# zellerlab/GECCO

Hardware: AMD Instinct MI355X
Metric: genes/sec CRF decode (windowed fwd-bwd marginals + Viterbi) (higher is better)
Workload: dtype f64

## Files before the change

gecco_amd/csrc/crf_kernels.hip:

```cpp
#include "crf_device.hpp"
#include "crf_vd_short.hpp"

namespace gecco {
namespace {

typedef double f64x2 __attribute__((ext_vector_type(2)));

__device__ __forceinline__ double wave_shr1_zero(double v) {
    int lo = __double2loint(v), hi = __double2hiint(v);
    lo = __builtin_amdgcn_update_dpp(0, lo, 0x138, 0xF, 0xF, true);
    hi = __builtin_amdgcn_update_dpp(0, hi, 0x138, 0xF, 0xF, true);
    return __hiloint2double(hi, lo);
}

__device__ __forceinline__ double max_nocanon(double a, double b) {
    double r;
    asm("v_max_f64 %0, %1, %2" : "=v"(r) : "v"(a), "v"(b));
    return r;
}

__device__ __forceinline__ int xcd_remap(int orig, int nwg) {
    const int xcd = orig & 7, q = nwg >> 3, r = nwg & 7;
    const int base = xcd < r ? xcd * (q + 1) : r * (q + 1) + (xcd - r) * q;
    return base + (orig >> 3);
}

__device__ __forceinline__ void store_wt(double *p, double v) {
    __hip_atomic_store(reinterpret_cast<unsigned long long *>(p), static_cast<unsigned long long>(__double_as_longlong(v)),
                       __ATOMIC_RELAXED, __HIP_MEMORY_SCOPE_AGENT);
}

__device__ __forceinline__ double lds_read1(const double *p) {
    return __longlong_as_double(static_cast<long long>(
        __hip_atomic_load(reinterpret_cast<const unsigned long long *>(p), __ATOMIC_RELAXED, __HIP_MEMORY_SCOPE_WORKGROUP)));
}

__device__ __forceinline__ void rescale_pair(double &u, double &v) {
    int ex;
    (void)frexp(fmax(u, v), &ex);
    u = ldexp(u, -ex);
    v = ldexp(v, -ex);
}


constexpr int kGatherUnroll = 8;

template <int WMAX, int NT, int TT, bool EXACT>
struct WinSmem {
    static constexpr int JMAX = TT == 1 ? 2 : TT;
    static constexpr int CAP = TT == 1 ? NT + WMAX - 1 : TT * NT;
    static constexpr int CMAX = EXACT ? CAP / WMAX + 3 : CAP + 2;
    f64x2 ef[2 * CAP];
    uint32_t ginfo[CAP];
    f64x2 carry[NT / 64][WMAX];
    int32_t cslot[CMAX];
    int32_t cgene[CMAX];
    int32_t cn[CMAX];
};

struct SlotInfo {
    int gene;
    bool start_ok;
};

template <class Smem>
__device__ __forceinline__ SlotInfo slot_lookup(const Smem &sm, int cnt, int q, int S, int W, int step) {
    SlotInfo r{-1, false};
    if (q < 0 || q >= S) return r;
    int lo = 0, hi = cnt - 1;
    while (lo < hi) {
        const int mid = (lo + hi + 1) >> 1;
        if (sm.cslot[mid] <= q) lo = mid; else hi = mid - 1;
    }
    const int pos = q - sm.cslot[lo];
    const int np = sm.cslot[lo + 1] - sm.cslot[lo];
    const int n = sm.cn[lo];
    const int gl = pos - ((np - n) >> 1);
    if (gl >= 0 && gl < n) r.gene = sm.cgene[lo] + gl;
    r.start_ok = (pos + W <= np) && (step == 1 || pos % step == 0);
    return r;
}

__device__ __forceinline__ void state_scores_l2(const int32_t *__restrict__ attr_id,
                                                const double2 *__restrict__ wtab2, int n_attrs, int lo, int hi,
                                                double &s0, double &s1) {
    for (int base = lo; base < hi; base += kGatherUnroll) {
        int a[kGatherUnroll];
#pragma unroll
        for (int u = 0; u < kGatherUnroll; ++u) a[u] = base + u < hi ? attr_id[base + u] : -1;
        double2 w[kGatherUnroll];
#pragma unroll
        for (int u = 0; u < kGatherUnroll; ++u) w[u] = unsigned(a[u]) < unsigned(n_attrs) ? wtab2[a[u]] : make_double2(0.0, 0.0);
#pragma unroll
        for (int u = 0; u < kGatherUnroll; ++u) {
            s0 += w[u].x;
            s1 += w[u].y;
        }
    }
}

typedef int i32x4 __attribute__((ext_vector_type(4)));

__device__ __forceinline__ void state_scores_buf(__amdgpu_buffer_rsrc_t ra, __amdgpu_buffer_rsrc_t rw, uint32_t off,
                                                 uint32_t cnt, double &s0, double &s1) {
    for (uint32_t base = 0; base < cnt; base += kGatherUnroll) {
        int a[kGatherUnroll];
#pragma unroll
        for (int u = 0; u < kGatherUnroll; ++u)
            a[u] = __builtin_amdgcn_raw_buffer_load_b32(ra, int((off + base + u) << 2), 0, 0);
        i32x4 w[kGatherUnroll];
#pragma unroll
        for (int u = 0; u < kGatherUnroll; ++u) {
            const uint32_t wo = base + u < cnt ? min(uint32_t(a[u]), 0x0FFFFFFFu) << 4 : 0xFFFFFFF0u;
            w[u] = __builtin_amdgcn_raw_buffer_load_b128(rw, int(wo), 0, 0);
        }
#pragma unroll
        for (int u = 0; u < kGatherUnroll; ++u) {
            s0 += __hiloint2double(w[u].y, w[u].x);
            s1 += __hiloint2double(w[u].w, w[u].z);
        }
    }
}

template <int WMAX, bool EXACT, bool RESCALE, int NT, int TT, bool LEAN = false, bool SMALL = false>
__device__ __forceinline__ void windowed_tile(const WinArgs &P, WinSmem<WMAX, NT, TT, EXACT> &sm, const int tile) {
    using Smem = WinSmem<WMAX, NT, TT, EXACT>;
    constexpr int JMAX = Smem::JMAX;
    constexpr bool RATIO = !RESCALE && EXACT;
    const int W = EXACT ? WMAX : P.W;
    const int tid = threadIdx.x, lane = tid & 63, wave = tid >> 6;
    const int OUT = NT - (W - 1);
    const int ns = TT * OUT + 2 * (W - 1);
    const int q0 = tile * (TT * OUT) - (W - 1);

    const int4 td = P.all_regular ? make_int4(0, 0, 0, 1) : P.tile_desc[tile];
    int gene[JMAX];
    bool start[JMAX];
#pragma unroll
    for (int j = 0; j < JMAX; ++j) {
        gene[j] = -1;
        start[j] = false;
    }
    if (td.w & 1) {
#pragma unroll
        for (int j = 0; j < JMAX; ++j) {
            const int sl = tid + j * NT, q = q0 + sl;
            if (sl < ns && q >= 0 && q < P.S) {
                gene[j] = q + td.x;
                start[j] = (reinterpret_cast<const uint32_t *>(P.start_bits)[q >> 5] >> (q & 31)) & 1u;
            }
        }
    } else {
        const int cnt = td.z - td.y + 1;
        for (int j = tid; j <= cnt; j += NT) {
            sm.cslot[j] = P.c_slot[td.y + j];
            if (j < cnt) {
                sm.cgene[j] = P.c_gene[td.y + j];
                sm.cn[j] = P.c_n[td.y + j];
            }
        }
        __syncthreads();
#pragma unroll
        for (int j = 0; j < JMAX; ++j) {
            const int sl = tid + j * NT;
            if (sl < ns) {
                const SlotInfo si = slot_lookup(sm, cnt, q0 + sl, P.S, W, P.step);
                gene[j] = si.gene;
                start[j] = si.start_ok;
            }
        }
    }

    const uint32_t nnz = SMALL ? uint32_t(P.csr_end) : uint32_t(P.gene_ptr[P.n_genes]);
    const int g_first = (td.w & 1) ? (q0 > 0 ? q0 : 0) + td.x : P.c_gene[td.y];
    const uint32_t lo_tile = SMALL ? uint32_t(P.csr_begin) : uint32_t(P.gene_ptr[g_first]);
    const uint64_t abytes = uint64_t(nnz - lo_tile) << 2;
    const __amdgpu_buffer_rsrc_t ra = __builtin_amdgcn_make_buffer_rsrc(
        const_cast<int32_t *>(P.attr_id + lo_tile), 0, abytes > 0xFFFFFFFFull ? 0xFFFFFFFFu : uint32_t(abytes), 0x00020000);
    const __amdgpu_buffer_rsrc_t rw =
        __builtin_amdgcn_make_buffer_rsrc(const_cast<double2 *>(P.wtab2), 0, uint32_t(P.A) << 4, 0x00020000);

    double sc0[JMAX], sc1[JMAX];
#pragma unroll
    for (int j = 0; j < JMAX; ++j) sc0[j] = sc1[j] = 0.0;
    if (td.w & 1) {
        uint32_t lo[JMAX], hi[JMAX];
#pragma unroll
        for (int j = 0; j < JMAX; ++j) {
            lo[j] = hi[j] = 0;
            if (gene[j] >= 0) {
                lo[j] = uint32_t(P.gene_ptr[gene[j]]);
                hi[j] = uint32_t(P.gene_ptr[gene[j] + 1]);
            }
        }
        const int q_end = min(q0 + ns, P.S);
        const uint32_t hi_tile = SMALL ? uint32_t(P.csr_end) : uint32_t(P.gene_ptr[q_end + td.x]);
        const uint32_t n_attr = hi_tile - lo_tile;
        constexpr int SBASE = (Smem::CAP + 1) / 2;
        constexpr int APL = (2 * Smem::CAP - SBASE) / NT;
        constexpr int SCAP = APL * NT;
        static_assert(APL >= 1, "parking area smaller than one round of the workgroup");
        f64x2 *park = sm.ef + SBASE;
#pragma unroll 1
        for (uint32_t base = 0; base < n_attr; base += SCAP) {
            int id[APL];
#pragma unroll
            for (int a = 0; a < APL; ++a) id[a] = __builtin_amdgcn_raw_buffer_load_b32(ra, int((base + a * NT + tid) << 2), 0, 0);
            i32x4 w[APL];
#pragma unroll
            for (int a = 0; a < APL; ++a) {
                const uint32_t wo = min(uint32_t(id[a]), 0x0FFFFFFFu) << 4;
                w[a] = __builtin_amdgcn_raw_buffer_load_b128(rw, int(wo), 0, 0);
            }
#pragma unroll
            for (int a = 0; a < APL; ++a)
                park[a * NT + tid] = f64x2{__hiloint2double(w[a].y, w[a].x), __hiloint2double(w[a].w, w[a].z)};
            __syncthreads();
            const uint32_t c0 = lo_tile + base, c1 = c0 + SCAP;
#pragma unroll
            for (int j = 0; j < JMAX; ++j) {
                const f64x2 *k = park + (max(lo[j], c0) - c0);
                const f64x2 *const e = park + (min(hi[j], c1) - c0);
                for (; k < e && hi[j] > c0; ++k) {
                    const f64x2 v = *k;
                    sc0[j] += v.x;
                    sc1[j] += v.y;
                }
            }
            if (base + SCAP < n_attr) __syncthreads();
        }
        if (!RATIO && n_attr > 0) __syncthreads();
    } else {
        uint32_t off[JMAX], cnt[JMAX];
#pragma unroll
        for (int j = 0; j < JMAX; ++j) {
            int lo = 0, hi = 0;
            if (gene[j] >= 0) {
                lo = P.gene_ptr[gene[j]];
                hi = P.gene_ptr[gene[j] + 1];
            }
            off[j] = uint32_t(lo) - lo_tile;
            cnt[j] = uint32_t(hi - lo);
        }
        int ids[JMAX][kGatherUnroll];
#pragma unroll
        for (int j = 0; j < JMAX; ++j)
            if (TT > 1 || j == 0 || wave == 0) {
#pragma unroll
                for (int u = 0; u < kGatherUnroll; ++u)
                    ids[j][u] = __builtin_amdgcn_raw_buffer_load_b32(ra, int((off[j] + u) << 2), 0, 0);
            }
#pragma unroll
        for (int j = 0; j < JMAX; ++j) {
            if (TT > 1 || j == 0 || wave == 0) {
                double s0 = 0.0, s1 = 0.0;
                i32x4 w[kGatherUnroll];
#pragma unroll
                for (int u = 0; u < kGatherUnroll; ++u) {
                    const uint32_t wo = uint32_t(u) < cnt[j] ? min(uint32_t(ids[j][u]), 0x0FFFFFFFu) << 4 : 0xFFFFFFF0u;
                    w[u] = __builtin_amdgcn_raw_buffer_load_b128(rw, int(wo), 0, 0);
                }
#pragma unroll
                for (int u = 0; u < kGatherUnroll; ++u) {
                    s0 += __hiloint2double(w[u].y, w[u].x);
                    s1 += __hiloint2double(w[u].w, w[u].z);
                }
                if (cnt[j] > uint32_t(kGatherUnroll))
                    state_scores_buf(ra, rw, off[j] + kGatherUnroll, cnt[j] - kGatherUnroll, s0, s1);
                sc0[j] = s0;
                sc1[j] = s1;
            }
        }
    }
    double *rr = reinterpret_cast<double *>(sm.ef);
#pragma unroll
    for (int j = 0; j < JMAX; ++j) {
        if (TT > 1 || j == 0 || wave == 0) {
            const int sl = tid + j * NT;
            const double s0 = sc0[j], s1 = sc1[j];
            if (sl >= W - 1 && sl < TT * OUT + (W - 1) && gene[j] >= 0) {
                if (P.state_out) reinterpret_cast<f64x2 *>(P.state_out)[gene[j]] = P.label ? f64x2{s0, s1} : f64x2{s1, s0};
            }
            const double d = s1 - s0;
            if (sl < ns) {
                if (RATIO) {
                    const double r = mu_exp_tab(d, P.rtab, P.expc);
                    rr[sl] = __hiloint2double(__double2hiint(r) | (start[j] ? int(0x80000000u) : 0), __double2loint(r));
                    if (!(td.w & 1)) sm.ginfo[sl] = uint32_t(gene[j] + 1);
                } else {
                    const double e = exp_neg(fabs(d), P.expc);
                    const double e1 = d > 0.0 ? 1.0 : e;
                    sm.ef[sl] = f64x2{d > 0.0 ? e : 1.0, P.mu01 * e1};
                    sm.ginfo[sl] = (start[j] ? 0x80000000u : 0u) | uint32_t(gene[j] + 1);
                }
            }
        }
    }
    if (P.dstate_out) {
#pragma unroll
        for (int j = 0; j < JMAX; ++j) {
            if (TT > 1 || j == 0 || wave == 0) {
                const int sl = tid + j * NT;
                if (sl >= W - 1 && sl < TT * OUT + (W - 1) && gene[j] >= 0) {
                    const double d = sc1[j] - sc0[j];
                    const double dd = __hiloint2double(__double2hiint(d) ^ (P.label ? 0 : int(0x80000000u)), __double2loint(d));
                    store_wt(P.dstate_out + gene[j], dd);
                }
            }
        }
    }
    __syncthreads();

    const uint32_t rmask = P.rescale_mask;
    const double rho = P.rho;
#pragma unroll 1
    for (int ph = 0; ph < TT; ++ph) {
        if (SMALL && ph > 0 && q0 + (W - 1) + ph * OUT >= P.S) break;
        const int sbase = ph * OUT + tid;
        bool my_start = false;
        int my_gene;
        if (RATIO) {
            const int q = q0 + sbase;
            my_gene = (td.w & 1) ? ((q >= 0 && q < P.S) ? q + td.x : -1) : int(sm.ginfo[sbase]) - 1;
        } else {
            const uint32_t gi = sm.ginfo[sbase];
            my_start = gi >> 31;
            my_gene = int(gi & 0x7fffffffu) - 1;
        }
        const f64x2 *ef = sm.ef + sbase;
        if constexpr (RATIO) {
            const double *rrs = rr + sbase;
            double A1[WMAX];
            const double r0 = lds_read1(rrs);
            double a0 = 1.0, a1 = fabs(r0) * P.kappa_over_mu01;
            A1[0] = a1;
#pragma unroll
            for (int k = 1; k < WMAX; ++k) {
                if (EXACT || k < W) {
                    const double r = fabs(lds_read1(rrs + k));
                    const double t = a0 + a1;
                    a1 = fma(a1, rho, a0) * r;
                    a0 = t;
                    A1[k] = a1;
                }
            }
            asm volatile("" ::: "memory");
            double z = fma(a1, P.inv_kappa, a0);
            const bool renorm = __builtin_amdgcn_ballot_w64(!(z < P.ratio_zmax)) != 0;
            auto pair_of = [&](double r, double &e0, double &f) {
                const bool pos = r > P.mu01;
                const double rc = fmin(r, 1.0e300);
                double q = __builtin_amdgcn_rcp(rc);
                q = fma(fma(-rc, q, 1.0), q, q);
                e0 = pos ? P.mu01 * q : 1.0;
                f = pos ? P.mu01 : r;
            };
            if (renorm) {
                double e0, f;
                pair_of(fabs(r0), e0, f);
                a0 = e0;
                a1 = f * P.kappa_over_mu01;
                A1[0] = a1;
#pragma unroll
                for (int k = 1; k < WMAX; ++k) {
                    if (EXACT || k < W) {
                        pair_of(fabs(rrs[k]), e0, f);
                        const double t = a0 + a1;
                        a1 = fma(a1, rho, a0) * f;
                        a0 = t * e0;
                        A1[k] = a1;
                    }
                }
                z = fma(a1, P.inv_kappa, a0);
            }
            double b0, b1;
            {
                double r = __builtin_amdgcn_rcp(z);
                r = fma(fma(-z, r, 1.0), r, r);
                b0 = __double2hiint(r0) < 0 ? r : 0.0;
                b1 = b0 * P.inv_kappa;
            }
            double R = 0.0;
            double *carry = reinterpret_cast<double *>(&sm.carry[0][0]);
            if (!renorm) {
                double rcur = W > 1 ? lds_read1(rrs + (W - 1)) : 0.0;
#pragma unroll
                for (int k = WMAX - 1; k >= 0; --k) {
                    if (EXACT || k < W) {
                        double rnext = 0.0;
                        if (k > 1) rnext = lds_read1(rrs + (k - 1));
                        const double cand = A1[k] * b1;
                        if (k < W - 1) {
                            if (lane == 63 && wave < NT / 64 - 1) carry[wave * WMAX + k] = R;
                            R = wave_shr1_zero(R);
                        }
                        R = max_nocanon(R, cand);
                        if (k > 0) {
                            const double u = fabs(rcur) * b1;
                            b1 = fma(u, rho, b0);
                            b0 = b0 + u;
                        }
                        rcur = rnext;
                    }
                }
            } else {
#pragma unroll
                for (int k = WMAX - 1; k >= 0; --k) {
                    if (EXACT || k < W) {
                        const double cand = A1[k] * b1;
                        if (k < W - 1) {
                            if (lane == 63 && wave < NT / 64 - 1) carry[wave * WMAX + k] = R;
                            R = wave_shr1_zero(R);
                        }
                        R = max_nocanon(R, cand);
                        if (k > 0) {
                            double e0, f;
                            pair_of(fabs(rrs[k]), e0, f);
                            const double cc = e0 * b0, u = f * b1;
                            b0 = cc + u;
                            b1 = fma(u, rho, cc);
                        }
                    }
                }
            }
            __syncthreads();
            if (wave > 0 && lane < W - 1) {
                int t2 = tid;
                if (LEAN) asm volatile("" : "+v"(t2));
                R = fmax(R, carry[((t2 >> 6) - 1) * WMAX + (t2 & 63)]);
            }
            R = fmin(R, 1.0);
            if (tid >= W - 1 && my_gene >= 0) store_wt(P.p_out + my_gene, R);
        } else if constexpr (!RESCALE) {
            double A1[WMAX];
            double a0, a1;
            {
                const f64x2 c = ef[0];
                a0 = c.x;
                a1 = fabs(c.y) * P.kappa_over_mu01;
            }
            A1[0] = a1;
#pragma unroll
            for (int k = 1; k < WMAX; ++k) {
                if (EXACT || k < W) {
                    const f64x2 c = ef[k];
                    const double t = a0 + a1;
                    a1 = fma(a1, rho, a0) * fabs(c.y);
                    a0 = t * c.x;
                    A1[k] = a1;
                }
            }
            asm volatile("" ::: "memory");

            double b0, b1;
            {
                const double z = fma(a1, P.inv_kappa, a0);
                double r = __builtin_amdgcn_rcp(z);
                r = fma(fma(-z, r, 1.0), r, r);
                b0 = my_start ? r : 0.0;
                b1 = b0 * P.inv_kappa;
            }
            double R = 0.0;
            double *carry = reinterpret_cast<double *>(&sm.carry[0][0]);
#pragma unroll
            for (int k = WMAX - 1; k >= 0; --k) {
                if (EXACT || k < W) {
                    const double cand = A1[k] * b1;
                    if (k < W - 1) {
                        if (lane == 63 && wave < NT / 64 - 1) carry[wave * WMAX + k] = R;
                        R = wave_shr1_zero(R);
                    }
                    R = max_nocanon(R, cand);
                    if (k > 0) {
                        const f64x2 c = ef[k];
                        const double cc = c.x * b0, u = fabs(c.y) * b1;
                        b0 = cc + u;
                        b1 = fma(u, rho, cc);
                    }
                }
            }
            __syncthreads();
            if (wave > 0 && lane < W - 1) R = fmax(R, carry[(wave - 1) * WMAX + lane]);
            R = fmin(R, 1.0);
            if (tid >= W - 1 && my_gene >= 0) P.p_out[my_gene] = R;
        } else {
            double A0[WMAX], A1[WMAX];
            double a0, a1;
            {
                const f64x2 c = ef[0];
                a0 = c.x;
                a1 = c.y * P.kappa_over_mu01;
            }
            A0[0] = a0;
            A1[0] = a1;
#pragma unroll
            for (int k = 1; k < WMAX; ++k) {
                if (EXACT || k < W) {
                    const f64x2 c = ef[k];
                    const double t = a0 + a1;
                    const double n1 = fma(a1, rho, a0) * c.y;
                    a0 = t * c.x;
                    a1 = n1;
                    if ((rmask >> k) & 1u) rescale_pair(a0, a1);
                    A0[k] = a0;
                    A1[k] = a1;
                }
            }
            asm volatile("" ::: "memory");
            double b0 = 1.0, b1 = P.inv_kappa;
            double Rx = 0.0, Ry = 0.0;
#pragma unroll
            for (int k = WMAX - 1; k >= 0; --k) {
                if (EXACT || k < W) {
                    const double x = A1[k] * b1;
                    const double y = A0[k] * b0;
                    if (k < W - 1) {
                        if (lane == 63 && wave < NT / 64 - 1) sm.carry[wave][k] = f64x2{Rx, Ry};
                        Rx = wave_shr1_zero(Rx);
                        Ry = wave_shr1_zero(Ry);
                    }
                    const bool take = my_start && (x * Ry >= Rx * y);
                    Rx = take ? x : Rx;
                    Ry = take ? y : Ry;
                    if (k > 0) {
                        const f64x2 c = ef[k];
                        const double cc = c.x * b0, u = c.y * b1;
                        b0 = cc + u;
                        b1 = fma(u, rho, cc);
                        if ((rmask >> k) & 1u) rescale_pair(b0, b1);
                    }
                }
            }
            __syncthreads();
            if (wave > 0 && lane < W - 1) {
                const f64x2 c = sm.carry[wave - 1][lane];
                if (c.x * Ry > Rx * c.y || (Rx == 0.0 && Ry == 0.0)) {
                    Rx = c.x;
                    Ry = c.y;
                }
            }
            if (tid >= W - 1 && my_gene >= 0) P.p_out[my_gene] = (Rx + Ry > 0.0) ? Rx / (Rx + Ry) : 0.0;
        }
        if (TT > 1) __syncthreads();
    }
}

template <int WMAX, bool EXACT, bool RESCALE, int NT, int TT>
__global__ void __launch_bounds__(NT, (RESCALE ? (WMAX <= 20 ? 5 : 3) : (WMAX <= 20 ? (TT <= 2 ? 8 : 5) : 3))) crf_windowed_l2(const WinArgs P) {
    __shared__ WinSmem<WMAX, NT, TT, EXACT> sm;
    windowed_tile<WMAX, EXACT, RESCALE, NT, TT>(P, sm, xcd_remap(blockIdx.x, P.ntiles));
}

__global__ void __launch_bounds__(kWinThreads, 4) crf_windowed_small_l2(const WinArgs P) {
    __shared__ WinSmem<20, kWinThreads, 2, true> sm;
    windowed_tile<20, true, false, kWinThreads, 2, false, true>(P, sm, 0);
}

struct PipeArgs {
    const int32_t *gene_ptr, *attr_id;
    const double2 *wtab2;
    const int32_t *c_slot, *c_gene, *c_n;
    const int4 *tile_desc;
    const uint64_t *start_bits;
    double *p_out, *dstate_out;
    const double *rtab;
    int32_t S, ntiles, step, label, n_genes, A, all_regular, nvd8;
    double mu01, rho, kappa_over_mu01, inv_kappa, ratio_zmax, expc5[5];
    const double *dstate;
    const uint8_t *flags;
    const uint16_t *lane_bits;
    const int32_t *cblk, *csr_gene_ptr, *csr_attr_id;
    const double2 *csr_wtab01;
    double2 *alpha;
    uint32_t *vd_stats;
    int8_t *y;
    int32_t s_n_genes, csr_n_attrs, v_exact, n_cblocks;
    double t00, t01, t10, t11, v_lo, v_hi, v_k, v_wmax2, v_tmax;
};

template <int TILES, int WGS>
__global__ void __launch_bounds__(kWinThreads, WGS) crf_decode_pipelined(const PipeArgs K) {
    using Smem = WinSmem<20, kWinThreads, TILES, true>;
    constexpr size_t kBytes = sizeof(Smem) > sizeof(VdShortSmem) ? sizeof(Smem) : sizeof(VdShortSmem);
    static_assert(kBytes <= 20480, "eight workgroups per CU");
    __shared__ __attribute__((aligned(16))) unsigned char raw[kBytes];
    const int b = blockIdx.x;
    if (b >= K.nvd8) {
        WinArgs P{};
        P.gene_ptr = K.gene_ptr;
        P.attr_id = K.attr_id;
        P.wtab2 = K.wtab2;
        P.c_slot = K.c_slot;
        P.c_gene = K.c_gene;
        P.c_n = K.c_n;
        P.tile_desc = K.tile_desc;
        P.start_bits = K.start_bits;
        P.p_out = K.p_out;
        P.dstate_out = K.dstate_out;
        P.rtab = K.rtab;
        P.S = K.S;
        P.ntiles = K.ntiles;
        P.W = 20;
        P.step = K.step;
        P.L = 2;
        P.label = K.label;
        P.n_genes = K.n_genes;
        P.A = K.A;
        P.tiles_per_wg = TILES;
        P.all_regular = K.all_regular;
        P.mu01 = K.mu01;
        P.rho = K.rho;
        P.kappa_over_mu01 = K.kappa_over_mu01;
        P.inv_kappa = K.inv_kappa;
        P.ratio_zmax = K.ratio_zmax;
#pragma unroll
        for (int i = 0; i < 5; ++i) P.expc[7 + i] = K.expc5[i];
        P.csr_begin = P.csr_end = -1;
        windowed_tile<20, true, false, kWinThreads, TILES, true>(P, *reinterpret_cast<Smem *>(raw), xcd_remap(b - K.nvd8, K.ntiles));
        return;
    }
    if (b >= K.n_cblocks) return;
    SeqArgs A{};
    A.dstate = K.dstate;
    A.flags = K.flags;
    A.lane_bits = K.lane_bits;
    A.cblk = K.cblk;
    A.csr_gene_ptr = K.csr_gene_ptr;
    A.csr_attr_id = K.csr_attr_id;
    A.csr_wtab01 = K.csr_wtab01;
    A.csr_n_attrs = K.csr_n_attrs;
    A.alpha = K.alpha;
    A.vd_stats = K.vd_stats;
    A.y = K.y;
    A.n_genes = K.s_n_genes;
    A.n_cblocks = K.n_cblocks;
    A.short_contigs = 1;
    A.v_exact = K.v_exact;
    A.t00 = K.t00;
    A.t01 = K.t01;
    A.t10 = K.t10;
    A.t11 = K.t11;
    A.v_lo = K.v_lo;
    A.v_hi = K.v_hi;
    A.v_k = K.v_k;
    A.v_wmax2 = K.v_wmax2;
    A.v_tmax = K.v_tmax;
    vd_short_block(A, b, *reinterpret_cast<VdShortSmem *>(raw));
}

__device__ __forceinline__ double2 slot_emission(const WinArgs &P, int gene) {
    double s0 = 0.0, s1 = 0.0;
    if (gene >= 0) state_scores_l2(P.attr_id, P.wtab2, P.A, P.gene_ptr[gene], P.gene_ptr[gene + 1], s0, s1);
    const double m = fmax(s0, s1);
    return make_double2(exp(s0 - m), exp(s1 - m));
}

__global__ void __launch_bounds__(256) crf_windowed_generic_l2(const WinArgs P) {
    const int q = blockIdx.x * 256 + threadIdx.x;
    if (q >= P.S) return;
    if (!((P.start_bits[q >> 6] >> (q & 63)) & 1ull)) return;
    int lo = 0, hi = P.K - 1;
    while (lo < hi) {
        const int mid = (lo + hi + 1) >> 1;
        if (P.c_slot[mid] <= q) lo = mid; else hi = mid - 1;
    }
    const int s0 = P.c_slot[lo], np = P.c_slot[lo + 1] - s0, n = P.c_n[lo], g0 = P.c_gene[lo];
    const int pos = q - s0, lpad = (np - n) >> 1;
    const int W = P.W;
    const size_t stride = size_t(P.S);
    double2 *scr = reinterpret_cast<double2 *>(P.scratch);
    auto gene_of = [&](int k) {
        const int gl = pos + k - lpad;
        return (gl >= 0 && gl < n) ? g0 + gl : -1;
    };
    const double m00 = P.g00, m01 = P.g01, m10 = P.g10, m11 = P.g11;
    double a0, a1;
    {
        const double2 e = slot_emission(P, gene_of(0));
        a0 = e.x;
        a1 = e.y;
    }
    scr[q] = make_double2(a0, a1);
    for (int k = 1; k < W; ++k) {
        const double2 e = slot_emission(P, gene_of(k));
        const double t0 = fma(a1, m10, a0 * m00), t1 = fma(a1, m11, a0 * m01);
        a0 = t0 * e.x;
        a1 = t1 * e.y;
        rescale_pair(a0, a1);
        scr[size_t(k) * stride + q] = make_double2(a0, a1);
    }
    double b0 = 1.0, b1 = 1.0;
    for (int k = W - 1; k >= 0; --k) {
        const double2 al = scr[size_t(k) * stride + q];
        const double x = al.y * b1, y = al.x * b0;
        const int gene = gene_of(k);
        if (gene >= 0) {
            const double pr = x / (x + y);
            atomicMax(reinterpret_cast<unsigned long long *>(P.p_out + gene), (unsigned long long)__double_as_longlong(pr));
        }
        if (k > 0) {
            const double2 e = slot_emission(P, gene);
            const double c0 = e.x * b0, c1 = e.y * b1;
            b0 = fma(m01, c1, m00 * c0);
            b1 = fma(m11, c1, m10 * c0);
            rescale_pair(b0, b1);
        }
    }
}

__global__ void fill_nan_kernel(double *p, const int2 *ranges, int n_ranges) {
    const int r = blockIdx.x * blockDim.x + threadIdx.x;
    if (r >= n_ranges) return;
    const int2 rg = ranges[r];
    const double nan = __longlong_as_double(0x7ff8000000000000LL);
    for (int g = rg.x; g < rg.y; ++g) p[g] = nan;
}

}

const char *windowed_kernel_name(int W, int L, bool fast) {
    if (L == 2 && fast && W == 20) return "crf_windowed_l2<20,exact>";
    if (L == 2 && fast && W <= kWinMaxW) return "crf_windowed_l2<32,dynamic>";
    if (L == 2) return "crf_windowed_generic_l2";
    return "unsupported";
}

int windowed_tile_out(int W, int L, int tt) {
    if (L == 2 && W <= kWinMaxW) return tt * (kWinThreads - (W - 1));
    return kWinThreads;
}

template <int TT>
static hipError_t launch_windowed_tt(const WinArgs &a, hipStream_t stream) {
    const dim3 grid(a.ntiles), block(kWinThreads);
    if (a.W == 20 && a.rescale_mask == 0) {
        hipLaunchKernelGGL((crf_windowed_l2<20, true, false, kWinThreads, TT>), grid, block, 0, stream, a);
    } else if (a.W == 20) {
        hipLaunchKernelGGL((crf_windowed_l2<20, true, true, kWinThreads, TT>), grid, block, 0, stream, a);
    } else if (a.rescale_mask == 0) {
        hipLaunchKernelGGL((crf_windowed_l2<kWinMaxW, false, false, kWinThreads, TT>), grid, block, 0, stream, a);
    } else {
        hipLaunchKernelGGL((crf_windowed_l2<kWinMaxW, false, true, kWinThreads, TT>), grid, block, 0, stream, a);
    }
    return hipGetLastError();
}

hipError_t launch_windowed(const WinArgs &a, hipStream_t stream) {
    if (a.ntiles <= 0) return hipSuccess;
    if (a.L == 2 && a.generic) {
        hipLaunchKernelGGL(crf_windowed_generic_l2, dim3((a.S + 255) / 256), dim3(256), 0, stream, a);
        return hipGetLastError();
    }
    if (a.L != 2 || a.W > kWinMaxW) return hipErrorNotSupported;
    if (a.ntiles == 1 && a.all_regular && a.csr_end >= 0 && a.csr_begin >= 0 && a.W == 20 && a.rescale_mask == 0 && a.tiles_per_wg == 2) {
        hipLaunchKernelGGL(crf_windowed_small_l2, dim3(1), dim3(kWinThreads), 0, stream, a);
        return hipGetLastError();
    }
    switch (a.tiles_per_wg) {
    case 1: return launch_windowed_tt<1>(a, stream);
    case 2: return launch_windowed_tt<2>(a, stream);
    case 3: return launch_windowed_tt<3>(a, stream);
    default: return hipErrorNotSupported;
    }
}

bool decode_pipelined_ok(const WinArgs &w, const SeqArgs &s) {
    return w.ntiles > 0 && w.W == 20 && w.rescale_mask == 0 && (w.tiles_per_wg == 1 || w.tiles_per_wg == 2) && !w.generic && w.L == 2 && !w.state_out &&
           s.short_contigs && s.n_cblocks > 0 && s.n_genes > 0;
}

hipError_t launch_decode_pipelined(const WinArgs &w, const SeqArgs &s, hipStream_t stream) {
    if (!decode_pipelined_ok(w, s)) return hipErrorNotSupported;
    PipeArgs k{};
    k.gene_ptr = w.gene_ptr;
    k.attr_id = w.attr_id;
    k.wtab2 = w.wtab2;
    k.c_slot = w.c_slot;
    k.c_gene = w.c_gene;
    k.c_n = w.c_n;
    k.tile_desc = w.tile_desc;
    k.start_bits = w.start_bits;
    k.p_out = w.p_out;
    k.dstate_out = w.dstate_out;
    k.rtab = w.rtab;
    k.S = w.S;
    k.ntiles = w.ntiles;
    k.step = w.step;
    k.label = w.label;
    k.n_genes = w.n_genes;
    k.A = w.A;
    k.all_regular = w.all_regular;
    k.nvd8 = (s.n_cblocks + 7) & ~7;
    k.mu01 = w.mu01;
    k.rho = w.rho;
    k.kappa_over_mu01 = w.kappa_over_mu01;
    k.inv_kappa = w.inv_kappa;
    k.ratio_zmax = w.ratio_zmax;
    for (int i = 0; i < 5; ++i) k.expc5[i] = w.expc[7 + i];
    k.dstate = s.dstate;
    k.flags = s.flags;
    k.lane_bits = s.lane_bits;
    k.cblk = s.cblk;
    k.csr_gene_ptr = s.csr_gene_ptr;
    k.csr_attr_id = s.csr_attr_id;
    k.csr_wtab01 = s.csr_wtab01;
    k.csr_n_attrs = s.csr_n_attrs;
    k.alpha = s.alpha;
    k.vd_stats = s.vd_stats;
    k.y = s.y;
    k.s_n_genes = s.n_genes;
    k.v_exact = s.v_exact;
    k.n_cblocks = s.n_cblocks;
    k.t00 = s.t00;
    k.t01 = s.t01;
    k.t10 = s.t10;
    k.t11 = s.t11;
    k.v_lo = s.v_lo;
    k.v_hi = s.v_hi;
    k.v_k = s.v_k;
    k.v_wmax2 = s.v_wmax2;
    k.v_tmax = s.v_tmax;
    if (w.tiles_per_wg == 1)
        hipLaunchKernelGGL((crf_decode_pipelined<1, 6>), dim3(k.nvd8 + w.ntiles), dim3(kWinThreads), 0, stream, k);
    else
        hipLaunchKernelGGL((crf_decode_pipelined<2, 8>), dim3(k.nvd8 + w.ntiles), dim3(kWinThreads), 0, stream, k);
    return hipGetLastError();
}

hipError_t launch_fill_nan(double *p, const int2 *ranges, int n_ranges, hipStream_t stream) {
    if (n_ranges <= 0) return hipSuccess;
    hipLaunchKernelGGL(fill_nan_kernel, dim3((n_ranges + 255) / 256), dim3(256), 0, stream, p, ranges, n_ranges);
    return hipGetLastError();
}

}
```

gecco_amd/csrc/crf_vd_short.hpp:

```cpp
#pragma once

#include "crf_device.hpp"
#include "crf_scan.hpp"

namespace gecco {
namespace {

constexpr int kT = 256;
constexpr int kGPL = kSeqGenesPerLane;
constexpr int kBlockGenes = kT * kGPL;
static_assert(kBlockGenes == kSeqBlockGenes, "host tables assume this block size");

__device__ __forceinline__ double vd_max(double a, double b) {
    double r;
    asm("v_max_f64 %0, %1, %2" : "=v"(r) : "v"(a), "v"(b));
    return r;
}
__device__ __forceinline__ double vd_min(double a, double b) {
    double r;
    asm("v_min_f64 %0, %1, %2" : "=v"(r) : "v"(a), "v"(b));
    return r;
}
__device__ __forceinline__ double vd_min_abs(double a, double b) {
    double r;
    asm("v_min_f64 %0, |%1|, |%2|" : "=v"(r) : "v"(a), "v"(b));
    return r;
}
__device__ __forceinline__ double vd_max_s(double a, double bound) {
    double r;
    asm("v_max_f64 %0, %1, %2" : "=v"(r) : "v"(a), "s"(bound));
    return r;
}
__device__ __forceinline__ double vd_min_s(double a, double bound) {
    double r;
    asm("v_min_f64 %0, %1, %2" : "=v"(r) : "v"(a), "s"(bound));
    return r;
}
__device__ __forceinline__ void vd_shift_in_gt(uint32_t &acc, double x, double bound) {
    asm("v_cmp_lt_f64 vcc, %2, %1\n\tv_addc_co_u32 %0, vcc, %0, %0, vcc" : "+v"(acc) : "v"(x), "s"(bound) : "vcc");
}
struct COp {
    static __device__ __forceinline__ CE identity() { return CE{0.0, -__builtin_huge_val(), __builtin_huge_val()}; }
    static __device__ __forceinline__ CE combine(const CE &a, const CE &b) {
        return CE{a.a + b.a, vd_min(vd_max(a.L + b.a, b.L), b.H), vd_min(vd_max(a.H + b.a, b.L), b.H)};
    }
    static __device__ __forceinline__ void combine_into(CE &t, CE &v) {
        asm volatile(
            "v_add_f64 %[tl], %[tl], %[a]\n\t"
            "v_add_f64 %[th], %[th], %[a]\n\t"
            "v_add_f64 %[a], %[ta], %[a]\n\t"
            "v_max_f64 %[tl], %[tl], %[L]\n\t"
            "v_max_f64 %[th], %[th], %[L]\n\t"
            "v_min_f64 %[L], %[tl], %[H]\n\t"
            "v_min_f64 %[H], %[th], %[H]"
            : [a] "+v"(v.a), [L] "+v"(v.L), [H] "+v"(v.H), [tl] "+v"(t.L), [th] "+v"(t.H)
            : [ta] "v"(t.a));
    }
};

__device__ __forceinline__ double vd_bound(const SeqArgs &A, double nnz, double n) { return nnz * A.v_wmax2 + (n + 2.0) * A.v_tmax; }
constexpr double kVdEps = 2.220446049250313e-16;
__device__ __forceinline__ double vd_margin(double r, double ulpM) { return (4.0 * r + 4.0) * ulpM; }

constexpr int kFixChunk = 1024;
struct FixStage {
    double2 st[kFixChunk];
    uint32_t bpw[kFixChunk / 16];
};
__device__ __forceinline__ void exact_states(const SeqArgs &A, int g0, int m, FixStage &fx, int first_lane) {
    const int nl = kT - first_lane, me = int(threadIdx.x) - first_lane;
    if (me < 0) return;
    for (int base = me; base < m; base += 4 * nl) {
        int lo[4], hi[4];
        double s0[4], s1[4];
        int longest = 0;
#pragma unroll
        for (int u = 0; u < 4; ++u) {
            const int i = base + u * nl;
            lo[u] = hi[u] = 0;
            if (i < m) {
                lo[u] = A.csr_gene_ptr[g0 + i];
                hi[u] = A.csr_gene_ptr[g0 + i + 1];
            }
            s0[u] = s1[u] = 0.0;
        }
#pragma unroll
        for (int u = 0; u < 4; ++u) longest = max(longest, hi[u] - lo[u]);
        for (int k = 0; k < longest; ++k) {
            int a[4];
#pragma unroll
            for (int u = 0; u < 4; ++u) a[u] = lo[u] + k < hi[u] ? A.csr_attr_id[lo[u] + k] : -1;
            double2 w[4];
#pragma unroll
            for (int u = 0; u < 4; ++u) w[u] = unsigned(a[u]) < unsigned(A.csr_n_attrs) ? A.csr_wtab01[a[u]] : make_double2(0.0, 0.0);
#pragma unroll
            for (int u = 0; u < 4; ++u) {
                s0[u] += w[u].x;
                s1[u] += w[u].y;
            }
        }
#pragma unroll
        for (int u = 0; u < 4; ++u) {
            const int i = base + u * nl;
            if (i < m) fx.st[i] = make_double2(s0[u], s1[u]);
        }
    }
}
__device__ __forceinline__ void exact_walk(const SeqArgs &A, FixStage &fx, int m, bool first, double &d0, double &d1) {
    int i = 0;
    if (first) {
        d0 = fx.st[0].x;
        d1 = fx.st[0].y;
        i = 1;
    }
    auto step = [&](const double2 s) {
        const double a0 = d0 + A.t00, b0 = d1 + A.t10;
        const double a1 = d0 + A.t01, b1 = d1 + A.t11;
        d0 = fmax(a0, b0) + s.x;
        d1 = fmax(a1, b1) + s.y;
    };
    for (; i < m && (i & 7); ++i) {
        step(fx.st[i]);
        fx.st[i] = make_double2(d0, d1);
    }
    for (; i + 8 <= m; i += 8) {
        double2 sv[8];
#pragma unroll
        for (int u = 0; u < 8; ++u) sv[u] = fx.st[i + u];
#pragma unroll
        for (int u = 0; u < 8; ++u) {
            step(sv[u]);
            fx.st[i + u] = make_double2(d0, d1);
        }
    }
    for (; i < m; ++i) {
        step(fx.st[i]);
        fx.st[i] = make_double2(d0, d1);
    }
}
__device__ __forceinline__ void exact_backpointers(const SeqArgs &A, FixStage &fx, int m, bool first, double e0, double e1) {
    for (int w = threadIdx.x; 16 * w < m; w += kT) {
        uint32_t word = 0;
        for (int i = max(16 * w, first ? 1 : 0); i < min(16 * w + 16, m); ++i) {
            const double p0 = i ? fx.st[i - 1].x : e0, p1 = i ? fx.st[i - 1].y : e1;
            const uint32_t arg0 = (p0 + A.t00) < (p1 + A.t10) ? 1u : 0u, arg1 = (p0 + A.t01) < (p1 + A.t11) ? 1u : 0u;
            word |= (arg0 | (arg1 << 1)) << (2 * (i & 15));
        }
        fx.bpw[w] = word;
    }
}
__device__ __forceinline__ uint32_t *exact_bp_words(const SeqArgs &A, int gs) { return reinterpret_cast<uint32_t *>(A.alpha) + size_t(gs); }
__device__ __forceinline__ uint32_t *exact_end_labels(const SeqArgs &A, int gs) {
    return reinterpret_cast<uint32_t *>(A.alpha) + size_t(A.n_genes) + size_t(gs);
}
__device__ __forceinline__ void exact_backtrack(const SeqArgs &A, int gs, int ge, double d0, double d1) {
    const int n = ge - gs, nw = (n + 15) / 16;
    uint32_t *bpc = exact_bp_words(A, gs), *endl = exact_end_labels(A, gs);
    auto word_map = [&](uint32_t bits, int w, uint32_t y) {
        const int hi = min(16 * w + 15, n - 1), lo = max(16 * w, 1);
        for (int t = hi; t >= lo; --t) y = (bits >> (2 * (t & 15) + y)) & 1u;
        return y;
    };
    for (int w = threadIdx.x; w < nw; w += kT) {
        const uint32_t bits = bpc[w];
        endl[w] = word_map(bits, w, 0) | (word_map(bits, w, 1) << 1);
    }
    __syncthreads();
    if (threadIdx.x == 0) {
        uint32_t y = d0 < d1 ? 1u : 0u;
        for (int w = nw - 1; w >= 0; --w) {
            const uint32_t mp = endl[w];
            endl[w] = y;
            y = (mp >> y) & 1u;
        }
    }
    __syncthreads();
    for (int w = threadIdx.x; w < nw; w += kT) {
        const uint32_t bits = bpc[w];
        uint32_t y = endl[w];
        const int hi = min(16 * w + 15, n - 1), lo = 16 * w;
        for (int t = hi; t >= lo; --t) {
            A.y[gs + t] = int8_t(y);
            if (t >= 1) y = (bits >> (2 * (t & 15) + y)) & 1u;
        }
    }
    __syncthreads();
}

__device__ __forceinline__ void exact_delta_contig(const SeqArgs &A, int gs, int ge, FixStage &fx) {
    uint32_t *bpc = exact_bp_words(A, gs);
    double d0 = 0.0, d1 = 0.0;
    for (int cb = gs; cb < ge; cb += kFixChunk) {
        const int m = min(kFixChunk, ge - cb);
        const double e0 = d0, e1 = d1;
        exact_states(A, cb, m, fx, 0);
        __syncthreads();
        if (threadIdx.x == 0) exact_walk(A, fx, m, cb == gs, d0, d1);
        __syncthreads();
        d0 = fx.st[m - 1].x;
        d1 = fx.st[m - 1].y;
        exact_backpointers(A, fx, m, cb == gs, e0, e1);
        __syncthreads();
        for (int i = threadIdx.x; i < (m + 15) / 16; i += kT) bpc[(cb - gs) / 16 + i] = fx.bpw[i];
        __syncthreads();
    }
    exact_backtrack(A, gs, ge, d0, d1);
}

constexpr double kVdPad = 1e30;

struct VdShortSmem {
    double st[kT * (kGPL + 1)];
    uint32_t mark[kBlockGenes / 32];
    int c_end;
    CE tot[kT / 64];
    uint32_t mtot[kT / 64];
    double pv[kT / 64];
    uint32_t pbad[kT / 64];
    uint32_t vote[kT / 64];
};
static_assert(sizeof(VdShortSmem) <= 20480, "eight workgroups per CU");
__device__ __forceinline__ void load_short(const double *__restrict__ v, int g0, int n, VdShortSmem &stg, double (&x)[kGPL]) {
    const int base = int(threadIdx.x) * kGPL;
    const double *vp = v + g0;
    double *row = stg.st + threadIdx.x * (kGPL + 1);
    const int wave_end = (__builtin_amdgcn_readfirstlane(int(threadIdx.x >> 6)) + 1) * 64 * kGPL;
    if (wave_end <= n) {
#pragma unroll
        for (int k = 0; k < kGPL; ++k) x[k] = vp[base + k];
#pragma unroll
        for (int k = 0; k < kGPL; ++k) row[k] = x[k];
        return;
    }
#pragma unroll
    for (int k = 0; k < kGPL; ++k) x[k] = vp[max(min(base + k, n - 1), 0)];
#pragma unroll
    for (int k = 0; k < kGPL; ++k) {
        x[k] = base + k < n ? x[k] : kVdPad;
        row[k] = x[k];
    }
}

__device__ __forceinline__ uint32_t wave_or_u32(uint32_t v) {
    v |= uint32_t(__builtin_amdgcn_update_dpp(0, int(v), 0x111, 0xF, 0xF, true));
    v |= uint32_t(__builtin_amdgcn_update_dpp(0, int(v), 0x112, 0xF, 0xF, true));
    v |= uint32_t(__builtin_amdgcn_update_dpp(0, int(v), 0x114, 0xF, 0xF, true));
    v |= uint32_t(__builtin_amdgcn_update_dpp(0, int(v), 0x118, 0xF, 0xF, true));
    v |= uint32_t(__builtin_amdgcn_update_dpp(0, int(v), 0x142, 0xA, 0xF, true));
    v |= uint32_t(__builtin_amdgcn_update_dpp(0, int(v), 0x143, 0xC, 0xF, true));
    return uint32_t(__builtin_amdgcn_readlane(int(v), 63));
}

constexpr int kVdRun = 6;
__device__ __forceinline__ void vd_apply(const CE &P, double in, double &v) {
    asm volatile("v_add_f64 %0, %1, %2\n\tv_max_f64 %0, %0, %3\n\tv_min_f64 %0, %0, %4" : "+v"(v) : "v"(in), "v"(P.a), "v"(P.L), "v"(P.H));
}
__device__ __forceinline__ void vd_propagate(const CE &P, double &v, uint64_t &known) {
    for (int it = 0; it < kVdRun; ++it) {
        const uint64_t todo = (known << 1) & ~known;
        if (!todo) break;
        const double in = dpp_f64_z<0x138>(v);
        if (__builtin_amdgcn_inverse_ballot_w64(todo)) vd_apply(P, in, v);
        known |= todo;
    }
}

__device__ __forceinline__ void vd_short_block(const SeqArgs &A, const int blk, VdShortSmem &stg) {
    CE *lds = stg.tot;
    uint32_t *ldsm = stg.mtot;
    const int slot = threadIdx.x;
    const int g0 = __builtin_amdgcn_readfirstlane(A.cblk[blk]), n = __builtin_amdgcn_readfirstlane(A.cblk[blk + 1]) - g0;
    const uint32_t bits = A.lane_bits[blk * kT + slot];
    const uint32_t first = bits & 0xffu, last = bits >> 8;
    const uint32_t wave_bits = wave_or_u32(bits);
    double x[kGPL];
    load_short(A.dstate, g0, n, stg, x);
    const int cnt = min(kGPL, n - slot * kGPL);
    const double *row = stg.st + slot * (kGPL + 1);
    CE P = COp::identity();
#pragma unroll
    for (int k = 0; k < kGPL; ++k) {
        const double dvk = x[k];
        const bool fst = (first >> k) & 1u;
        const double c = A.v_k + dvk;
        const double l2 = vd_min_s(vd_max_s(P.L, A.v_lo), A.v_hi) + c, h2 = vd_min_s(vd_max_s(P.H, A.v_lo), A.v_hi) + c;
        P.a += c;
        P.L = l2;
        P.H = h2;
        if ((wave_bits >> k) & 1u) {
            asm volatile("" ::: "memory");
            P.L = fst ? dvk : l2;
            P.H = fst ? dvk : h2;
        }
    }
    double Din;
    {
        const int wave = __builtin_amdgcn_readfirstlane(int(threadIdx.x >> 6));
        double v = P.L;
        uint64_t known = __builtin_amdgcn_ballot_w64(P.L == P.H);
        vd_propagate(P, v, known);
        const bool wave_bad = (known | (known - 1)) != ~uint64_t(0) || !(known & (wave ? (uint64_t(2) << kVdRun) - 1 : uint64_t(1)));
        if ((threadIdx.x & 63) == 63) stg.pv[wave] = v;
        block_or_post(wave_bad, stg.pbad);
        __syncthreads();
        if (block_or_read(stg.pbad)) {
            const CE M = block_scan_exclusive<COp, false, CE, kScanThreads, true, true>(P, lds, static_cast<CE *>(nullptr));
            Din = M.L;
        } else {
            const double carry = stg.pv[wave ? wave - 1 : 0];
            if (!(known & 1u)) {
                if ((threadIdx.x & 63) == 0) vd_apply(P, carry, v);
                known |= 1u;
                vd_propagate(P, v, known);
            }
            Din = dpp_f64<0x138, 0xF>(carry, v);
        }
    }
    double ulpM = 0.0, margin = 1e-6 * fmax(1.0, fmax(fabs(A.v_lo), fabs(A.v_hi)));
    if (A.csr_gene_ptr) {
        ulpM = vd_bound(A, double(A.csr_gene_ptr[g0 + n] - A.csr_gene_ptr[g0]), double(n)) * kVdEps;
        margin = vd_margin(double(n), ulpM);
    }
    ulpM = __hiloint2double(__builtin_amdgcn_readfirstlane(__double2hiint(ulpM)), __builtin_amdgcn_readfirstlane(__double2loint(ulpM)));
    margin = __hiloint2double(__builtin_amdgcn_readfirstlane(__double2hiint(margin)), __builtin_amdgcn_readfirstlane(__double2loint(margin)));
    uint32_t maps = 0, lane_map;
    bool sensitive = false;
    {
        double Dq = Din, nearest = __builtin_huge_val();
#pragma unroll
        for (int k = 0; k < kGPL; ++k) {
            const double dvk = row[k];
            const double stepped = vd_min_s(vd_max_s(Dq, A.v_lo), A.v_hi) + (A.v_k + dvk);
            Dq = stepped;
            if ((wave_bits >> k) & 1u) {
                asm volatile("" ::: "memory");
                Dq = ((first >> k) & 1u) ? dvk : stepped;
            }
            vd_shift_in_gt(maps, Dq, A.v_lo);
            vd_shift_in_gt(maps, Dq, A.v_hi);
            double dist = vd_min_abs(Dq - A.v_hi, Dq - A.v_lo);
            if ((wave_bits >> (8 + k)) & 1u) {
                asm volatile("" ::: "memory");
                const bool lst = (last >> k) & 1u;
                maps = lst ? ((maps & ~3u) | (Dq > 0.0 ? 3u : 0u)) : maps;
                dist = lst ? fabs(Dq) : dist;
            }
            nearest = vd_min(nearest, dist);
        }
        sensitive = nearest <= margin;
    }
    auto label_map = [&]() {
        uint32_t y0 = 0u, y1 = 1u;
#pragma unroll
        for (int k = kGPL - 1; k >= 0; --k) {
            y0 = __builtin_amdgcn_ubfe(maps, uint32_t(2 * (kGPL - 1 - k)) | y0, 1u);
            y1 = __builtin_amdgcn_ubfe(maps, uint32_t(2 * (kGPL - 1 - k)) | y1, 1u);
        }
        return y0 | (y1 << 1);
    };
    const bool lane_sensitive = sensitive && A.v_exact;
    int vote = lane_sensitive ? 1 : 0;
    uint32_t mtotal;
    lane_map = label_map();
    uint32_t lab = block_scan_exclusive_back<MapOp>(lane_map, ldsm, &mtotal, &vote, stg.vote) & 1u;
    const bool wg_sensitive = vote != 0;
    if (wg_sensitive) {
        double Dq = Din;
        uint64_t sat = 0;
#pragma unroll
        for (int k = 0; k < kGPL; ++k) {
            if (k < cnt) {
                const double dvk = row[k];
            Dq = ((first >> k) & 1u) ? dvk : fmin(fmax(Dq, A.v_lo), A.v_hi) + (A.v_k + dvk);
                const uint64_t c = Dq >= A.v_hi + margin ? 1u : (Dq <= A.v_lo - margin ? 2u : 0u);
                sat |= c << (8 * k);
            }
        }
        *reinterpret_cast<uint64_t *>(&stg.st[slot * (kGPL + 1) + kGPL]) = sat;
        __syncthreads();
    } else {
        sensitive = false;
    }
    bool lane_flagged = false;
    if (sensitive && cnt > 0) {
        double D = 0.0;
        int r = 0;
        auto certain = [&](double x) { return x >= A.v_hi + margin || x <= A.v_lo - margin; };
        if (!(first & 1u)) {
            const int t0 = slot * kGPL;
            int p = t0 - 1;
            auto dval = [&](int t) { return stg.st[(t / kGPL) * (kGPL + 1) + t % kGPL]; };
            for (;; --p) {
                if (A.flags[g0 + p] & 1u) {
                    D = dval(p);
                    r = 0;
                    break;
                }
                const uint32_t c = reinterpret_cast<const uint8_t *>(&stg.st[((p - 1) / kGPL) * (kGPL + 1) + kGPL])[(p - 1) % kGPL];
                if (c) {
                    D = (c == 1u ? A.v_hi : A.v_lo) + (A.v_k + dval(p));
                    r = 1;
                    break;
                }
            }
            for (int t = p + 1; t < t0; ++t) {
                r = certain(D) ? 1 : r + 1;
                D = fmin(fmax(D, A.v_lo), A.v_hi) + (A.v_k + dval(t));
            }
        }
        maps = 0;
#pragma unroll
        for (int k = 0; k < kGPL; ++k) {
            if (k < cnt) {
                const double dvk = row[k];
                const bool fst = (first >> k) & 1u;
                r = fst ? 0 : (certain(D) ? 1 : r + 1);
                D = fst ? dvk : fmin(fmax(D, A.v_lo), A.v_hi) + (A.v_k + dvk);
                const bool lst = (last >> k) & 1u;
                const double thi = lst ? 0.0 : A.v_hi, tlo = lst ? 0.0 : A.v_lo;
                maps |= ((D > thi ? 1u : 0u) | (D > tlo ? 2u : 0u)) << (2 * (kGPL - 1 - k));
                const double mr = vd_margin(double(r), ulpM);
                lane_flagged |= fabs(D - thi) <= mr || fabs(D - tlo) <= mr;
            }
        }
        if (A.vd_stats) {
            atomicAdd(A.vd_stats + 0, 1u);
            if (lane_flagged) atomicAdd(A.vd_stats + 1, 1u);
        }
    }
    bool wg_flagged = false;
    if (wg_sensitive) {
        block_or_post(lane_flagged, stg.vote);
        __syncthreads();
        wg_flagged = block_or_read(stg.vote);
        lane_map = label_map();
        lab = block_scan_exclusive_back<MapOp>(lane_map, ldsm, &mtotal) & 1u;
    }
    uint64_t packed = 0;
#pragma unroll
    for (int k = kGPL - 1; k >= 0; --k) {
        lab = __builtin_amdgcn_ubfe(maps, uint32_t(2 * (kGPL - 1 - k)) | lab, 1u);
        packed |= uint64_t(lab) << (8 * k);
    }
    {
        struct __attribute__((packed)) Bytes8 {
            uint64_t v;
        };
        int8_t *yp = A.y + g0 + slot * kGPL;
        if (cnt >= kGPL) {
            reinterpret_cast<Bytes8 *>(yp)->v = packed;
        } else {
            for (int k = 0; k < cnt; ++k) yp[k] = int8_t(packed >> (8 * k));
        }
    }
    if (wg_flagged && A.csr_gene_ptr) {
        uint32_t *mark = stg.mark;
        int *c_end = &stg.c_end;
        __syncthreads();
        if (slot < kBlockGenes / 32) mark[slot] = 0;
        __syncthreads();
        if (lane_flagged) {
            int prev = -1;
            for (int k = 0; k < cnt; ++k) {
                int t = slot * kGPL + k;
                while (!(A.flags[g0 + t] & 1u)) --t;
                if (t != prev) atomicOr(&mark[t >> 5], 1u << (t & 31));
                prev = t;
            }
        }
        __syncthreads();
        FixStage &st2 = *reinterpret_cast<FixStage *>(stg.st);
        static_assert(sizeof(stg.st) >= sizeof(FixStage), "exact pass: LDS for one chunk of state scores");
        for (int wi = 0; wi < kBlockGenes / 32; ++wi) {
            uint32_t bits = mark[wi];
            while (bits) {
                const int cs = wi * 32 + __builtin_ctz(bits);
                bits &= bits - 1;
                if (slot == 0) *c_end = n;
                __syncthreads();
                for (int i = cs + slot; i < n; i += kT)
                    if (A.flags[g0 + i] & 2u) {
                        atomicMin(c_end, i + 1);
                        break;
                    }
                __syncthreads();
                const int ce = *c_end;
                __syncthreads();
                if (slot == 0 && A.vd_stats) {
                    atomicAdd(A.vd_stats + 2, 1u);
                    atomicAdd(A.vd_stats + 3, uint32_t(ce - cs));
                }
                exact_delta_contig(A, g0 + cs, g0 + ce, st2);
            }
        }
    }
}

}
}
```

Baseline: 76.45 billion.

## Streamline regular-tile RATIO path: wave-level start masks, contiguous gene addressing, exec-masked sign

For regular tiles on the RATIO path, each wave now loads one 64-bit start mask and sets the sign bit under an exec mask, replacing the per-thread bit extraction. Gene pointer, state output and probability stores use contiguous base-plus-lane byte offsets with unsigned range checks instead of per-thread gene indices. The fmax/fmin clamp is replaced with non-canonicalizing v_max/v_min asm. A compile flag can hardwire regular tiles, and the exact-pass flag scan in the Viterbi code is rewritten with a scalar base pointer. The aim is to cut VALU address arithmetic and scattered loads in the scoring and store phases, in exchange for more inline asm and more complex code paths.

```diff
diff --git a/gecco_amd/csrc/crf_kernels.hip b/gecco_amd/csrc/crf_kernels.hip
--- a/gecco_amd/csrc/crf_kernels.hip
+++ b/gecco_amd/csrc/crf_kernels.hip
@@ -1,3 +1,5 @@
+#include <type_traits>
+
 #include "crf_device.hpp"
 #include "crf_vd_short.hpp"
 
@@ -33,6 +35,44 @@
 __device__ __forceinline__ double lds_read1(const double *p) {
     return __longlong_as_double(static_cast<long long>(
         __hip_atomic_load(reinterpret_cast<const unsigned long long *>(p), __ATOMIC_RELAXED, __HIP_MEMORY_SCOPE_WORKGROUP)));
+}
+
+__device__ __forceinline__ double clamp1_nocanon(double a) {
+    double r;
+    asm("v_min_f64 %0, %1, 1.0" : "=v"(r) : "v"(a));
+    return r;
+}
+
+__device__ __forceinline__ uint64_t start_mask64(const uint64_t *__restrict__ bits, int q) {
+    const uint64_t *w = bits + (q >> 6);
+    const uint64_t a = w[0], b = w[1];
+    const int sh = q & 63;
+    return sh ? (a >> sh) | (b << (64 - sh)) : a;
+}
+
+__device__ __forceinline__ int or_sign_if(int hi, uint64_t mask) {
+    uint64_t saved;
+    asm("s_mov_b64 %1, exec\n\ts_and_b64 exec, exec, %2\n\tv_or_b32 %0, 0x80000000, %0\n\ts_mov_b64 exec, %1"
+        : "+v"(hi), "=&s"(saved)
+        : "s"(mask)
+        : "scc");
+    return hi;
+}
+
+__device__ __forceinline__ bool in_range(int x, int lo, int len) { return uint32_t(x - lo) < uint32_t(len); }
+
+template <int SHIFT, bool PINNED = false>
+__device__ __forceinline__ uint32_t lane_offset(int tid) {
+    uint32_t r;
+    if (PINNED)
+        asm volatile("v_lshlrev_b32 %0, %1, %2" : "=v"(r) : "n"(SHIFT), "v"(tid));
+    else
+        asm("v_lshlrev_b32 %0, %1, %2" : "=v"(r) : "n"(SHIFT), "v"(tid));
+    return r;
+}
+template <class T>
+__device__ __forceinline__ T *at_bytes(T *base, uint32_t off) {
+    return reinterpret_cast<T *>(reinterpret_cast<char *>(const_cast<typename std::remove_const<T>::type *>(base)) + off);
 }
 
 __device__ __forceinline__ void rescale_pair(double &u, double &v) {
@@ -133,7 +173,11 @@
     const int ns = TT * OUT + 2 * (W - 1);
     const int q0 = tile * (TT * OUT) - (W - 1);
 
+#ifdef GECCO_CRF_REGULAR_TILES_ONLY
+    const int4 td = make_int4(0, 0, 0, 1);
+#else
     const int4 td = P.all_regular ? make_int4(0, 0, 0, 1) : P.tile_desc[tile];
+#endif
     int gene[JMAX];
     bool start[JMAX];
 #pragma unroll
@@ -141,7 +185,20 @@
         gene[j] = -1;
         start[j] = false;
     }
-    if (td.w & 1) {
+    const bool fast1 = RATIO && (td.w & 1);
+    const int g_base = q0 + td.x;
+    const int s_lo = max(0, -q0), s_hi = min(ns, P.S - q0), s_len = max(0, s_hi - s_lo);
+    const int o_lo = max(s_lo, W - 1), o_len = max(0, min(s_hi, TT * OUT + (W - 1)) - o_lo);
+    constexpr int NS_C = TT * (NT - (WMAX - 1)) + 2 * (WMAX - 1);
+    uint64_t smask[JMAX];
+#pragma unroll
+    for (int j = 0; j < JMAX; ++j) smask[j] = 0;
+    if (RATIO && (td.w & 1)) {
+        const int wv = __builtin_amdgcn_readfirstlane(wave);
+#pragma unroll
+        for (int j = 0; j < JMAX; ++j)
+            if (TT > 1 || j == 0 || wv == 0) smask[j] = start_mask64(P.start_bits, q0 + j * NT + wv * 64);
+    } else if (td.w & 1) {
 #pragma unroll
         for (int j = 0; j < JMAX; ++j) {
             const int sl = tid + j * NT, q = q0 + sl;
@@ -185,10 +242,19 @@
     for (int j = 0; j < JMAX; ++j) sc0[j] = sc1[j] = 0.0;
     if (td.w & 1) {
         uint32_t lo[JMAX], hi[JMAX];
+        const int32_t *const gp = P.gene_ptr + g_base;
+        const uint32_t t4 = RATIO ? lane_offset<2>(tid) : 0u;
 #pragma unroll
         for (int j = 0; j < JMAX; ++j) {
             lo[j] = hi[j] = 0;
-            if (gene[j] >= 0) {
+            if (RATIO) {
+                const int sl = tid + j * NT;
+                if (in_range(sl, s_lo, s_len)) {
+                    const int32_t *const b = at_bytes(gp + j * NT, t4);
+                    lo[j] = uint32_t(b[0]);
+                    hi[j] = uint32_t(b[1]);
+                }
+            } else if (gene[j] >= 0) {
                 lo[j] = uint32_t(P.gene_ptr[gene[j]]);
                 hi[j] = uint32_t(P.gene_ptr[gene[j] + 1]);
             }
@@ -273,9 +339,42 @@
         }
     }
     double *rr = reinterpret_cast<double *>(sm.ef);
+    if constexpr (RATIO) {
+        if (fast1) {
+            double dd[JMAX];
+            const uint32_t t8 = lane_offset<3>(tid);
+#pragma unroll
+            for (int j = 0; j < JMAX; ++j) {
+                if (TT > 1 || j == 0 || wave == 0) {
+                    const int sl = tid + j * NT;
+                    dd[j] = sc1[j] - sc0[j];
+                    if ((j + 1) * NT <= NS_C || sl < ns) {
+                        const double r = mu_exp_tab(dd[j], P.rtab, P.expc);
+                        *at_bytes(rr + j * NT, t8) = __hiloint2double(or_sign_if(__double2hiint(r), smask[j]), __double2loint(r));
+                    }
+                }
+            }
+            if (P.state_out || P.dstate_out) {
+                f64x2 *const so = reinterpret_cast<f64x2 *>(P.state_out) + g_base;
+                double *const dso = P.dstate_out + g_base;
+                const int flip = P.label ? 0 : int(0x80000000u);
+#pragma unroll
+                for (int j = 0; j < JMAX; ++j) {
+                    if (TT > 1 || j == 0 || wave == 0) {
+                        const int sl = tid + j * NT;
+                        if (in_range(sl, o_lo, o_len)) {
+                            if (P.state_out) so[uint32_t(sl)] = P.label ? f64x2{sc0[j], sc1[j]} : f64x2{sc1[j], sc0[j]};
+                            if (P.dstate_out)
+                                store_wt(at_bytes(dso + j * NT, t8), __hiloint2double(__double2hiint(dd[j]) ^ flip, __double2loint(dd[j])));
+                        }
+                    }
+                }
+            }
+        }
+    }
 #pragma unroll
     for (int j = 0; j < JMAX; ++j) {
-        if (TT > 1 || j == 0 || wave == 0) {
+        if (!fast1 && (TT > 1 || j == 0 || wave == 0)) {
             const int sl = tid + j * NT;
             const double s0 = sc0[j], s1 = sc1[j];
             if (sl >= W - 1 && sl < TT * OUT + (W - 1) && gene[j] >= 0) {
@@ -296,7 +395,7 @@
             }
         }
     }
-    if (P.dstate_out) {
+    if (P.dstate_out && !fast1) {
 #pragma unroll
         for (int j = 0; j < JMAX; ++j) {
             if (TT > 1 || j == 0 || wave == 0) {
@@ -318,10 +417,8 @@
         if (SMALL && ph > 0 && q0 + (W - 1) + ph * OUT >= P.S) break;
         const int sbase = ph * OUT + tid;
         bool my_start = false;
-        int my_gene;
+        int my_gene = -1;
         if (RATIO) {
-            const int q = q0 + sbase;
-            my_gene = (td.w & 1) ? ((q >= 0 && q < P.S) ? q + td.x : -1) : int(sm.ginfo[sbase]) - 1;
         } else {
             const uint32_t gi = sm.ginfo[sbase];
             my_start = gi >> 31;
@@ -427,10 +524,16 @@
             if (wave > 0 && lane < W - 1) {
                 int t2 = tid;
                 if (LEAN) asm volatile("" : "+v"(t2));
-                R = fmax(R, carry[((t2 >> 6) - 1) * WMAX + (t2 & 63)]);
-            }
-            R = fmin(R, 1.0);
-            if (tid >= W - 1 && my_gene >= 0) store_wt(P.p_out + my_gene, R);
+                R = max_nocanon(R, carry[((t2 >> 6) - 1) * WMAX + (t2 & 63)]);
+            }
+            R = clamp1_nocanon(R);
+            if (td.w & 1) {
+                const int e_lo = max(W - 1, s_lo - ph * OUT), e_len = max(0, s_hi - ph * OUT - e_lo);
+                if (in_range(tid, e_lo, e_len)) store_wt(at_bytes(P.p_out + (g_base + ph * OUT), lane_offset<3, true>(tid)), R);
+            } else {
+                my_gene = int(sm.ginfo[ph * OUT + tid]) - 1;
+                if (tid >= W - 1 && my_gene >= 0) store_wt(P.p_out + my_gene, R);
+            }
         } else if constexpr (!RESCALE) {
             double A1[WMAX];
             double a0, a1;
diff --git a/gecco_amd/csrc/crf_vd_short.hpp b/gecco_amd/csrc/crf_vd_short.hpp
--- a/gecco_amd/csrc/crf_vd_short.hpp
+++ b/gecco_amd/csrc/crf_vd_short.hpp
@@ -474,13 +474,15 @@
         for (int wi = 0; wi < kBlockGenes / 32; ++wi) {
             uint32_t bits = mark[wi];
             while (bits) {
-                const int cs = wi * 32 + __builtin_ctz(bits);
+                int cs = wi * 32 + __builtin_ctz(bits), nn = n, sl = slot;
+                asm volatile("" : "+s"(cs), "+s"(nn), "+v"(sl));
                 bits &= bits - 1;
-                if (slot == 0) *c_end = n;
+                if (slot == 0) *c_end = nn;
                 __syncthreads();
-                for (int i = cs + slot; i < n; i += kT)
-                    if (A.flags[g0 + i] & 2u) {
-                        atomicMin(c_end, i + 1);
+                const uint8_t *const fl = A.flags + (g0 + cs);
+                for (int i = sl; cs + i < n; i += kT)
+                    if (fl[i] & 2u) {
+                        atomicMin(c_end, cs + i + 1);
                         break;
                     }
                 __syncthreads();
```

Result: no change. 76.61 billion (median of 2 runs) (+0.2%).
